# nv-tlabs/ChronoEdit

Measured on AMD Instinct MI355X. Metric: denoising-steps/sec, higher is better.
Workload: dtype bf16

## Files before the change

### chronoedit_amd/csrc/ce_attn.hip

```cpp
#include <cstdlib>

#include "ce_common.h"

namespace {

constexpr int HD = 128;
constexpr int QW = 32;
constexpr int KVB = 64;
constexpr int K_TILE_BYTES = KVB * HD * 2;
constexpr int VT_TILE_BYTES = HD * KVB * 2;
constexpr int BUF_BYTES = K_TILE_BYTES + VT_TILE_BYTES;
constexpr int OST_ROW = HD * 2 + 16;
constexpr int smem_bytes(int nwave, bool two_seg) {
  const int stage = nwave * QW * OST_ROW;
  return two_seg ? 2 * BUF_BYTES + stage : (stage > 2 * BUF_BYTES ? stage : 2 * BUF_BYTES);
}
constexpr float NEG_BIG = -1.0e30f;

__device__ __forceinline__ int vt_swz(int dv) {
  return ((((dv >> 2) & 7) << 1) | (((dv >> 1) ^ (dv >> 5)) & 1)) ^ (((dv >> 6) & 1) << 1);
}

struct KVSeg {
  const bf16* k;
// ... 220 lines not shown
          w1 = pack_bf16(bf16lo(pv[1]) + bf16lo(w1), bf16hi(pv[1]) + bf16hi(w1));
        }
        u32x2 val = {w0, w1};
        *slot = val;
      }
  }

  __syncthreads();
#pragma unroll
  for (int i = 0; i < 8; ++i) {
    const int c = lane + 64 * i;
    const int rl = c >> 4, cc = c & 15;
    const int q = q0 + rl;
    if (q < Nq) {
      const u32x4 v = *reinterpret_cast<const u32x4*>(smem + (TWO_SEG ? 2 * BUF_BYTES : 0) + (size_t)(wave * QW + rl) * OST_ROW + cc * 16);
      *reinterpret_cast<u32x4*>(O + (size_t)q * ldo + hoff + cc * 8) = v;
    }
  }
}


#define CE_EPOCH_BARRIER()                          \
  asm volatile("s_waitcnt lgkmcnt(0)" ::: "memory"); \
  __builtin_amdgcn_s_barrier()
constexpr int PK_ROW = HD * 2 + 16;
constexpr int PV_ROW = KVB * 2 + 16;
constexpr int PK_TILE = KVB * PK_ROW;
constexpr int PV_TILE = HD * PV_ROW;
typedef __attribute__((ext_vector_type(4))) unsigned pp_u4;
typedef __attribute__((ext_vector_type(2))) unsigned pp_u2;

constexpr int K_GRP = 1088;
typedef __attribute__((address_space(3))) void lds_void;
#ifdef CE_DIAGNOSTICS
__device__ unsigned long long g_sp_exact_hits = 0ull;
#endif
constexpr float SP_SPEC_THR = 1024.0f;
constexpr int SP_V0 = 2 * PK_TILE;
constexpr int SP_TILE_BYTES = 2 * PK_TILE + 3 * PV_TILE;
constexpr int sp_smem_bytes(bool two_seg) { return two_seg ? SP_TILE_BYTES + 8 * QW * OST_ROW : SP_TILE_BYTES; }

template <bool TWO_SEG, bool VT = false, bool QOUT = false, bool WGT = false>
__global__ __launch_bounds__(512, 2) void attn_fwd_sp_kernel(const bf16* __restrict__ Q_, bf16* __restrict__ O_, KVSeg seg0_,
                                                              KVSeg seg1_, int Nq, int H, int ldq, int ldo, int nqb,
                                                              float scale_log2e, int batch, BlkRows blk) {
  extern __shared__ __attribute__((aligned(16))) unsigned char smem[];
  constexpr int NWAVE = 8, QB = QW * NWAVE;
  const int tid = threadIdx.x, lane = tid & 63;
  const int wave = __builtin_amdgcn_readfirstlane(tid >> 6);
  const int l31 = lane & 31, hh = lane >> 5;
  for (int item = blockIdx.x; item < nqb * H * batch; item += gridDim.x) {
  const bf16* Q = Q_;
  bf16* O = O_;
  KVSeg seg0 = seg0_, seg1 = seg1_;

  int head, qb, bz;
  {
    const int nqb_full = Nq / QB;
    if ((H & 7) == 0) {
      const int xcd = item & 7, local = item >> 3, hx_n = H >> 3;
      const int full = batch * hx_n * nqb_full;
      if (local < full) {
        bz = local / (hx_n * nqb_full);
        const int r = local % (hx_n * nqb_full);
        head = xcd + 8 * (r / nqb_full);
        qb = r % nqb_full;
      } else {
        const int l2 = local - full;
        bz = l2 / hx_n;
        head = xcd + 8 * (l2 % hx_n);
        qb = nqb_full;
      }
    } else {
      bz = item / (nqb * H);
      const int r = item % (nqb * H);
      head = r / nqb;
      qb = r % nqb;
    }
  }
  {
    if (VT && blk.rows > 0) {
      Q += (size_t)bz * blk.rows * ldq;
      O += (size_t)bz * blk.rows * ldo;
      seg0.k += (size_t)bz * blk.rows * seg0.ldk;
      seg0.v += (size_t)bz * blk.vt_cols;
    } else if (TWO_SEG && VT) {
      Q += (size_t)bz * blk.q_rows * ldq;
      O += (size_t)bz * Nq * ldo;
      seg0.k += (size_t)bz * blk.k0_rows * seg0.ldk;
      seg0.v += (size_t)bz * blk.vt_cols;
    } else {
      Q += (size_t)bz * Nq * ldq;
      O += (size_t)bz * Nq * ldo;
      seg0.k += (size_t)bz * seg0.len * seg0.ldk;
      seg0.v += VT ? (size_t)bz * (TWO_SEG ? blk.vt_cols : seg0.len) : (size_t)bz * seg0.len * seg0.ldv;
    }
    if (TWO_SEG) {
      seg1.k += (size_t)bz * (VT ? blk.k1_rows : seg1.len) * seg1.ldk;
      seg1.v += VT ? (size_t)bz * blk.stride : (size_t)bz * seg1.len * seg1.ldv;
    }
  }
  const int q0 = qb * QB + wave * QW;
  const int hoff = head * HD;
  const bool active = q0 < Nq;
  const int q0row = (VT && blk.rows > 0) ? (q0 / blk.rows) * blk.stride + q0 % blk.rows : q0;

  bf16x8 qf[8];
  {
    const bf16* qrow = Q + (size_t)(q0 + l31 < Nq ? q0row + l31 : 0) * ldq + hoff + 8 * hh;
#pragma unroll
    for (int ks = 0; ks < 8; ++ks) qf[ks] = *reinterpret_cast<const bf16x8*>(qrow + 16 * ks);
  }
  auto scale_q = [&]() __attribute__((always_inline)) {
#pragma unroll
  for (int ks = 0; ks < 8; ++ks) {
    const u32x4 w = __builtin_bit_cast(u32x4, qf[ks]);
    u32x4 o;
#pragma unroll
    for (int i = 0; i < 4; ++i) o[i] = pack_bf16(bf16lo(w[i]) * scale_log2e, bf16hi(w[i]) * scale_log2e);
    qf[ks] = __builtin_bit_cast(bf16x8, o);
  }
#pragma unroll
  for (int ks = 0; ks < 8; ++ks) asm volatile("" : "+v"(qf[ks]));

  };
  const int v_dvq = (tid & 1) | (((tid >> 4) & 15) << 1), v_kvq = ((tid >> 1) & 7) | (((tid >> 8) & 1) << 3);
  const int v_chunk = (v_kvq & ~3) | ((v_kvq & 1) << 1) | ((v_kvq >> 1) & 1);
  unsigned char* ost = smem + (TWO_SEG ? SP_TILE_BYTES : 0) + (size_t)(wave * QW + l31) * OST_ROW;
  const int k_w = l31 & 3;
  const unsigned char* k_rd = smem + (l31 >> 2) * K_GRP + k_w * 256 + ((hh ^ (k_w & 1)) << 4);
  const int k_eo[2] = {(k_w >> 1) << 5, ((k_w >> 1) ^ 1) << 5};
  const unsigned char* v_rd = smem + SP_V0 + l31 * PV_ROW + hh * 16;
  int vt_off[4];
#pragma unroll
  for (int s4 = 0; s4 < 4; ++s4) {
    const int x = (l31 >> 1) & 7;
    vt_off[s4] = l31 * 128 + ((2 * (s4 ^ (x >> 1)) + (hh ^ (x & 1))) << 4);
  }
  unsigned char* v_wr = smem + SP_V0 + (4 * v_dvq) * PV_ROW + v_chunk * 8;

#pragma unroll
  for (int sidx = 0; sidx < (TWO_SEG ? 2 : 1); ++sidx) {
    KVSeg sg = sidx == 0 ? seg0 : seg1;
    float w_last = 0.f;
    if (WGT && sidx == 0) {
      sg.len = min(max(blk.valid0[bz], 1), sg.len);
      w_last = blk.w0[bz];
    }
    const int ntiles = (sg.len + KVB - 1) / KVB;
    const int k_rows_span = (VT && blk.rows > 0) ? ((sg.len - 1) / blk.rows) * blk.stride + blk.rows : sg.len;
    const auto k_rsrc = __builtin_amdgcn_make_buffer_rsrc((void*)(sg.k + hoff), 0, (k_rows_span - 1) * sg.ldk * 2 + HD * 2, 0x00020000);
    const auto v_rsrc = VT ? __builtin_amdgcn_make_buffer_rsrc((void*)(sg.v + (size_t)hoff * sg.ldv), 0, ((HD - 1) * sg.ldv + ntiles * KVB) * 2, 0x00020000)
                           : __builtin_amdgcn_make_buffer_rsrc((void*)(sg.v + hoff), 0, (sg.len - 1) * sg.ldv * 2 + HD * 2, 0x00020000);
    int v_voff[4];
#pragma unroll
    for (int i = 0; i < 4; ++i) v_voff[i] = (4 * v_kvq + i) * sg.ldv * 2 + v_dvq * 8;
    const int k_tile_bytes = KVB * sg.ldk * 2, v_tile_bytes = KVB * sg.ldv * 2;

    f32x16 oacc[4];
#pragma unroll
    for (int m = 0; m < 4; ++m)
#pragma unroll
      for (int r = 0; r < 16; ++r) oacc[m][r] = 0.f;
    float l_run = 0.f, alpha_prev = 1.0f, mc = 0.f;
    f32x16 cinit;
#pragma unroll
    for (int r = 0; r < 16; ++r) cinit[r] = 0.f;
    u32x4 ppk[4];
#pragma unroll
    for (int s4 = 0; s4 < 4; ++s4) ppk[s4] = u32x4{0u, 0u, 0u, 0u};

    pp_u2 vreg[4];
    const int kd_row = VT ? (lane >> 4) + 4 * ((wave >> 1) & 1) + 8 * (wave & 1) + 16 * (wave >> 2) : 4 * wave + (lane >> 4);
    const int kd_voff0 = kd_row * sg.ldk * 2 + (((lane & 15) ^ (lane >> 4)) << 4), kd_voff1 = kd_voff0 + 32 * sg.ldk * 2;
    const int vd_row = 8 * wave + (lane >> 3);
    const int vd_voff0 = vd_row * sg.ldv * 2 + (((lane & 7) ^ ((vd_row >> 1) & 7)) << 4), vd_voff1 = vd_voff0 + 64 * sg.ldv * 2;
    auto dma_v = [&](int t, int buf, int j) {
      __builtin_amdgcn_raw_ptr_buffer_load_lds(v_rsrc, (lds_void*)(smem + SP_V0 + buf * PV_TILE + (wave + 8 * j) * 1024), 16,
                                               j ? vd_voff1 : vd_voff0, t * (KVB * 2), 0, 0);
    };
    auto dma_k = [&](int t, int buf, int j) {
      int soff = t * k_tile_bytes;
      if (VT && blk.rows > 0) {
        const int b_ = blk.magic ? (int)__umulhi((uint32_t)t, blk.magic) : t;
        soff = (b_ * blk.stride + (t - b_ * (blk.rows >> 6)) * KVB) * sg.ldk * 2;
      }
      __builtin_amdgcn_raw_ptr_buffer_load_lds(k_rsrc, (lds_void*)(smem + buf * PK_TILE + (wave + 8 * j) * K_GRP), 16,
                                               j ? kd_voff1 : kd_voff0, soff, 0, 0);
    };
    auto load_v = [&](int t) {
      const int so = t * v_tile_bytes;
#pragma unroll
      for (int i = 0; i < 4; ++i) vreg[i] = __builtin_amdgcn_raw_buffer_load_b64(v_rsrc, v_voff[i], so, 0);
    };
    auto store_v_part = [&](int buf, int j) {
      const int w = j >> 1;
      uint32_t lo, hi;
      if ((j & 1) == 0) {
        lo = (vreg[0][w] & 0xffffu) | (vreg[1][w] << 16);
        hi = (vreg[2][w] & 0xffffu) | (vreg[3][w] << 16);
      } else {
        lo = (vreg[0][w] >> 16) | (vreg[1][w] & 0xffff0000u);
        hi = (vreg[2][w] >> 16) | (vreg[3][w] & 0xffff0000u);
      }
      pp_u2 val = {lo, hi};
      *reinterpret_cast<pp_u2*>(v_wr + buf * PV_TILE + j * PV_ROW) = val;
    };
    auto store_v = [&](int buf) {
#pragma unroll
      for (int j = 0; j < 4; ++j) {
        const int w = j >> 1;
        uint32_t lo, hi;
        if ((j & 1) == 0) {
          lo = (vreg[0][w] & 0xffffu) | (vreg[1][w] << 16);
          hi = (vreg[2][w] & 0xffffu) | (vreg[3][w] << 16);
        } else {
          lo = (vreg[0][w] >> 16) | (vreg[1][w] & 0xffff0000u);
          hi = (vreg[2][w] >> 16) | (vreg[3][w] & 0xffff0000u);
        }
        pp_u2 val = {lo, hi};
        *reinterpret_cast<pp_u2*>(v_wr + buf * PV_TILE + j * PV_ROW) = val;
      }
    };

    if (TWO_SEG && sidx == 1) { CE_EPOCH_BARRIER(); }
    dma_k(0, 0, 0);
    dma_k(0, 0, 1);
    __builtin_amdgcn_sched_barrier(0);
    if (VT) {
      dma_v(0, 0, 0);
      dma_v(0, 0, 1);
    } else {
      load_v(0);
    }
    {
      const pp_u4 z = {0u, 0u, 0u, 0u};
      for (int i = tid; i < PV_TILE / 16; i += NWAVE * 64) *reinterpret_cast<pp_u4*>(smem + SP_V0 + 2 * PV_TILE + i * 16) = z;
    }
    if (!VT) {
      store_v(0);
      asm volatile("s_waitcnt vmcnt(0)" ::: "memory");
      load_v(1);
    }
    if (sidx == 0) scale_q();

#define CE_SP_KWAIT()                                          \
  do {                                                         \
    if (VT) asm volatile("s_waitcnt vmcnt(2)" ::: "memory");   \
    else asm volatile("s_waitcnt vmcnt(4)" ::: "memory");      \
  } while (0)
    int vb_prev = 2, vb_cur = 0;

    for (int t = 0; !active && t < ntiles; ++t) {
      CE_SP_KWAIT();
      CE_EPOCH_BARRIER();
      const int vb_next = 3 - vb_prev - vb_cur;
      dma_k(t + 1, (t + 1) & 1, 0);
      dma_k(t + 1, (t + 1) & 1, 1);
      __builtin_amdgcn_sched_barrier(0);
      if (VT) {
        dma_v(t + 1, vb_next, 0);
        dma_v(t + 1, vb_next, 1);
      } else {
        store_v(vb_next);
        load_v(t + 2);
      }
      vb_prev = vb_cur;
      vb_cur = vb_next;
    }
    for (int t = 0; active && t < ntiles; ++t) {
      CE_SP_KWAIT();
      CE_EPOCH_BARRIER();
      const int vb_next = 3 - vb_prev - vb_cur;
      const unsigned char* kb = k_rd + (t & 1) * PK_TILE;
      const unsigned char* vb = v_rd + vb_prev * PV_TILE;
      const unsigned char* vtb = smem + SP_V0 + vb_prev * PV_TILE;

      const f32x16 zero16 = {0.f, 0.f, 0.f, 0.f, 0.f, 0.f, 0.f, 0.f, 0.f, 0.f, 0.f, 0.f, 0.f, 0.f, 0.f, 0.f};
      f32x16 st[2];
      {
        constexpr int RING = VT ? 4 : 6;
        bf16x8 kf[RING];
#define CE_LDK(i) (*reinterpret_cast<const bf16x8*>(kb + k_eo[((i) >> 1) & 1] + ((i) & 1) * 8 * K_GRP + ((i) >> 2) * 64))
#pragma unroll
        for (int i = 0; i < RING; ++i) kf[i] = CE_LDK(i);
#pragma unroll
        for (int i = 0; i < 16; ++i) {
          if (i < 2) {
            asm("v_mfma_f32_32x32x16_bf16 %0, %1, %2, %3" : "=&v"(st[i & 1]) : "v"(kf[i % RING]), "v"(qf[i >> 1]), "v"(cinit));
          } else {
            st[i & 1] = __builtin_amdgcn_mfma_f32_32x32x16_bf16(kf[i % RING], qf[i >> 1], st[i & 1], 0, 0, 0);
          }
          if (i + RING < 16) kf[i % RING] = CE_LDK(i + RING);
          if (i == 1) dma_k(t + 1, (t + 1) & 1, 0);
          if (i == 3) dma_k(t + 1, (t + 1) & 1, 1);
          if (VT) {
            if (i == 5) dma_v(t + 1, vb_next, 0);
            if (i == 7) dma_v(t + 1, vb_next, 1);
          } else {
            if (i == 12) load_v(t + 2);
            if (i >= 5 && i < 9) store_v_part(vb_next, i - 5);
          }
          __builtin_amdgcn_sched_barrier(0);
        }
#undef CE_LDK
      }
      float alpha = 1.0f;
      float psum = 0.f;
      auto mask_tail = [&]() {
        if ((t + 1) * KVB > sg.len) {
          int thr = sg.len - t * KVB - (VT ? 8 : 4) * hh;
          asm volatile("" : "+v"(thr));
#pragma unroll
          for (int f = 0; f < 2; ++f)
#pragma unroll
            for (int r = 0; r < 16; ++r) {
              const int c = VT ? 32 * f + 16 * (r >> 3) + 4 * ((r >> 2) & 1) + (r & 3)
                               : 32 * f + (r & 3) + 8 * (r >> 2);
              if (c >= thr) st[f][r] = NEG_BIG;
            }
        }
      };
      auto weigh_last = [&]() {
        if (WGT && sidx == 0 && t == ntiles - 1 && w_last != 0.f) {
          int pos = sg.len - 1 - t * KVB - 8 * hh;
          asm volatile("" : "+v"(pos));
#pragma unroll
          for (int f = 0; f < 2; ++f)
#pragma unroll
            for (int r = 0; r < 16; ++r) {
              const int c = 32 * f + 16 * (r >> 3) + 4 * ((r >> 2) & 1) + (r & 3);
// ... 62 lines not shown
          __builtin_amdgcn_sched_barrier(0);
        }
        psum += st[1][14];
        psum += st[1][15];
#pragma unroll
        for (int j = 12; j < 16; ++j) pack_pair(j);
#undef CE_LDV
      }
      if (__builtin_expect(t > 0 && __any(psum > SP_SPEC_THR), 0)) {
        CE_DIAG_COUNT_EXACT(g_sp_exact_hits);
#pragma unroll
        for (int i = 0; i < 16; ++i) {
          const bf16x8 kfr = *reinterpret_cast<const bf16x8*>(kb + k_eo[(i >> 1) & 1] + (i & 1) * 8 * K_GRP + (i >> 2) * 64);
          st[i & 1] = __builtin_amdgcn_mfma_f32_32x32x16_bf16(kfr, qf[i >> 1], i < 2 ? zero16 : st[i & 1], 0, 0, 0);
        }
#pragma unroll
        for (int f = 0; f < 2; ++f)
#pragma unroll
          for (int r = 0; r < 16; ++r) st[f][r] -= mc;
        mask_tail();
        weigh_last();
        rebase();
        psum = 0.f;
#pragma unroll
        for (int j = 0; j < 16; ++j) {
          st[j >> 3][(2 * j) & 15] = __builtin_amdgcn_exp2f(st[j >> 3][(2 * j) & 15]);
          st[j >> 3][(2 * j + 1) & 15] = __builtin_amdgcn_exp2f(st[j >> 3][(2 * j + 1) & 15]);
          psum += st[j >> 3][(2 * j) & 15] + st[j >> 3][(2 * j + 1) & 15];
          pack_pair(j);
        }
      }
      l_run = l_run * alpha + psum;
      alpha_prev = alpha;
      vb_prev = vb_cur;
      vb_cur = vb_next;
    }
    if (active && __any(alpha_prev != 1.0f)) {
#pragma unroll
      for (int m = 0; m < 4; ++m)
#pragma unroll
        for (int r = 0; r < 16; ++r) oacc[m][r] *= alpha_prev;
    }
    if (VT) {
      asm volatile("s_waitcnt vmcnt(0)" ::: "memory");
      __builtin_amdgcn_s_barrier();
    }
    if (active) {
      const unsigned char* vb = v_rd + vb_prev * PV_TILE;
      const unsigned char* vtb = smem + SP_V0 + vb_prev * PV_TILE;
#pragma unroll
      for (int u = 0; u < 16; ++u) {
        const bf16x8 vfd = VT ? *reinterpret_cast<const bf16x8*>(vtb + vt_off[u >> 2] + (u & 3) * 4096)
                              : *reinterpret_cast<const bf16x8*>(vb + (u & 3) * 32 * PV_ROW + (u >> 2) * 32);
        oacc[u & 3] = __builtin_amdgcn_mfma_f32_32x32x16_bf16(vfd, __builtin_bit_cast(bf16x8, ppk[u >> 2]), oacc[u & 3], 0, 0, 0);
      }
    }
    CE_EPOCH_BARRIER();

    const float l_tot = l_run + __shfl_xor(l_run, 32, 64);
    const float inv = 1.0f / l_tot;
#pragma unroll
    for (int m = 0; m < 4; ++m)
#pragma unroll
      for (int a = 0; a < 4; ++a) {
        uint32_t w0 = pack_bf16(oacc[m][4 * a + 0] * inv, oacc[m][4 * a + 1] * inv);
        uint32_t w1 = pack_bf16(oacc[m][4 * a + 2] * inv, oacc[m][4 * a + 3] * inv);
        u32x2* slot = reinterpret_cast<u32x2*>(ost + (32 * m + 8 * a + 4 * hh) * 2);
        if (TWO_SEG && sidx == 1) {
          const u32x2 pv = *slot;
          w0 = pack_bf16(bf16lo(pv[0]) + bf16lo(w0), bf16hi(pv[0]) + bf16hi(w0));
          w1 = pack_bf16(bf16lo(pv[1]) + bf16lo(w1), bf16hi(pv[1]) + bf16hi(w1));
        }
        u32x2 val = {w0, w1};
        *slot = val;
      }
  }

  if (TWO_SEG && VT && QOUT) {
    const int ktiles = (H * HD) >> 7;
    const int grow = bz * Nq + q0 + l31;
#pragma unroll
    for (int m = 0; m < 4; ++m) {
      uint32_t pk[8];
      float amax = 0.f;
#pragma unroll
      for (int a = 0; a < 4; ++a) {
        const u32x2 pv = *reinterpret_cast<const u32x2*>(ost + (32 * m + 8 * a + 4 * hh) * 2);
        pk[2 * a] = pv[0];
        pk[2 * a + 1] = pv[1];
        amax = fmaxf(amax, fmaxf(fmaxf(fabsf(bf16lo(pv[0])), fabsf(bf16hi(pv[0]))), fmaxf(fabsf(bf16lo(pv[1])), fabsf(bf16hi(pv[1])))));
      }
      amax = fmaxf(amax, __shfl_xor(amax, 32, 64));
      const int byte = mx_scale_byte_nosat(amax);
      const float is = mx_inv_scale(byte);
#pragma unroll
      for (int a = 0; a < 4; ++a) {
        int w = 0;
        w = __builtin_amdgcn_cvt_pk_fp8_f32(clamp448(bf16lo(pk[2 * a]) * is), clamp448(bf16hi(pk[2 * a]) * is), w, false);
        w = __builtin_amdgcn_cvt_pk_fp8_f32(clamp448(bf16lo(pk[2 * a + 1]) * is), clamp448(bf16hi(pk[2 * a + 1]) * is), w, true);
        *reinterpret_cast<uint32_t*>(ost + 32 * m + 8 * a + 4 * hh) = (uint32_t)w;
      }
      if (hh == 0 && q0 + l31 < Nq) blk.s8[mx_gemm_scale_offset(grow, head * 4 + m, ktiles)] = (unsigned char)byte;
    }
    __syncthreads();
    unsigned char* O8 = blk.q8 + (size_t)bz * Nq * blk.ld8;
#pragma unroll
    for (int i = 0; i < 4; ++i) {
      const int c = lane + 64 * i;
      const int rl = c >> 3, cc = c & 7;
      if (q0 + rl < Nq) {
        const u32x4 v = *reinterpret_cast<const u32x4*>(smem + SP_TILE_BYTES + (size_t)(wave * QW + rl) * OST_ROW + cc * 16);
        *reinterpret_cast<u32x4*>(O8 + (size_t)(q0 + rl) * blk.ld8 + hoff + cc * 16) = v;
      }
    }
  } else {
  __syncthreads();
#pragma unroll
  for (int i = 0; i < 8; ++i) {
    const int c = lane + 64 * i;
    const int rl = c >> 4, cc = c & 15;
    if (q0 + rl < Nq) {
      const u32x4 v = *reinterpret_cast<const u32x4*>(smem + (TWO_SEG ? SP_TILE_BYTES : 0) + (size_t)(wave * QW + rl) * OST_ROW + cc * 16);
      *reinterpret_cast<u32x4*>(O + (size_t)(q0row + rl) * ldo + hoff + cc * 8) = v;
    }
  }
  }
  __syncthreads();
  }
}


#define W4A_S_FIRST(ST, KF, QF, CI) asm volatile("v_mfma_f32_32x32x16_bf16 %0, %1, %2, %3" : "=&v"(ST) : "v"(KF), "a"(QF), "v"(CI))
#define W4A_S(ST, KF, QF) asm volatile("v_mfma_f32_32x32x16_bf16 %0, %1, %2, %0" : "+v"(ST) : "v"(KF), "a"(QF))
#define W4A_PV(OA, VF, PP) asm volatile("v_mfma_f32_32x32x16_bf16 %0, %1, %2, %0" : "+a"(OA) : "v"(VF), "v"(PP))
#define W4A_ADD(ACC, X) asm volatile("v_add_f32 %0, %0, %1" : "+v"(ACC) : "v"(X))
#define W4A_CVT(DST, A, B)                                                                  \
  do {                                                                                      \
    uint32_t w_;                                                                            \
    asm volatile("v_cvt_pk_bf16_f32 %0, %1, %2" : "=v"(w_) : "v"(A), "v"(B));               \
    (DST) = w_;                                                                             \
  } while (0)
#ifndef W4_KDMA_IN_PV
#define W4_KDMA_IN_PV 1
#endif
#ifndef W4_ABLATE
#define W4_ABLATE 0
#endif
#ifndef W4_EXP_ASM
#define W4_EXP_ASM 1
#endif
#if W4_EXP_ASM
#define W4A_EXP(X) asm volatile("v_exp_f32 %0, %0" : "+v"(X))
#else
#define W4A_EXP(X) (X) = __builtin_amdgcn_exp2f(X)
#endif
#define W4A_SETTLE_S(SB) asm volatile("s_nop 11" : "+v"(st[SB][0]), "+v"(st[SB][1]))
#define W4A_SETTLE_O(SB) asm volatile("s_nop 11" : "+a"(oacc[SB][0]), "+a"(oacc[SB][1]), "+a"(oacc[SB][2]), "+a"(oacc[SB][3]))
constexpr int W4_KB = 4;
constexpr int W4_V0 = W4_KB * PK_TILE;
constexpr int W4_SMEM = W4_V0 + 3 * PV_TILE;
template <int N>
struct w4_int {
// ... 459 lines not shown
#ifdef CE_DIAGNOSTICS
extern "C" int ce_diag_mx_exact_hits(unsigned long long* out, int reset);
CE_API int ce_diag_attention_exact_route_hits(unsigned long long* hits, int reset) {
  if (!hits) return CE_ERR_ARG;
  unsigned long long v = 0ull, z = 0ull;
  if (hipDeviceSynchronize() != hipSuccess) return CE_ERR_ARG;
  if (hipMemcpyFromSymbol(&v, HIP_SYMBOL(g_sp_exact_hits), sizeof(v)) != hipSuccess) return CE_ERR_ARG;
  if (reset && hipMemcpyToSymbol(HIP_SYMBOL(g_sp_exact_hits), &z, sizeof(z)) != hipSuccess) return CE_ERR_ARG;
  hits[0] = v;
  return ce_diag_mx_exact_hits(hits + 1, reset);
}
#endif
CE_KNOB g_attn_nwave = 0;
#ifdef CE_DIAGNOSTICS
CE_API int ce_set_attention_waves(int nwave) {
  const int old = g_attn_nwave;
  if (nwave == 0 || nwave == 4 || nwave == 8 || nwave == 16 || nwave == 64 || nwave == 128 || nwave == 129) g_attn_nwave = nwave;
  return old;
}
#endif

CE_API int ce_attention_batched_bf16(const void* Q, const void* K1, const void* V1, int len1, int ldk1, int ldv1,
                                         const void* K2, const void* V2, int len2, int ldk2, int ldv2, void* O, int Nq, int H,
                                         int head_dim, int ldq, int ldo, float softmax_scale, int batch, hipStream_t stream) {
  if (!Q || !K1 || !V1 || !O) return CE_ERR_ARG;
  if (head_dim != HD || Nq <= 0 || H <= 0 || len1 <= 0 || batch <= 0 || batch > 65535) return CE_ERR_SHAPE;
  if ((ldq & 7) || (ldo & 7) || (ldk1 & 7) || (ldv1 & 3)) return CE_ERR_ALIGN;
  const bool two = (K2 != nullptr && V2 != nullptr && len2 > 0);
  if (two && ((ldk2 & 7) || (ldv2 & 3))) return CE_ERR_ALIGN;
  KVSeg s0{(const bf16*)K1, (const bf16*)V1, len1, ldk1, ldv1};
  KVSeg s1{(const bf16*)K2, (const bf16*)V2, two ? len2 : 0, ldk2, ldv2};
  const float sl2 = softmax_scale * 1.4426950408889634f;
  const bool sp = g_attn_nwave == 64 || g_attn_nwave == 0 || g_attn_nwave >= 128;
  const int nwave = sp ? 8 : g_attn_nwave;
  const int nqb = (Nq + nwave * QW - 1) / (nwave * QW);
  dim3 grid(nqb * H, batch), block(nwave * 64);
  if (sp) {
#define CE_ATTN_SP(TWO)                                                                                              \
  do {                                                                                                               \
    static bool done_[CE_MAX_DEVICES] = {};                                                                          \
    bool& done = done_[ce_device_slot()];                                                                            \
    if (!done) {                                                                                                     \
      (void)hipFuncSetAttribute((const void*)attn_fwd_sp_kernel<TWO>, hipFuncAttributeMaxDynamicSharedMemorySize,    \
                                sp_smem_bytes(TWO));                                                                 \
      done = true;                                                                                                   \
    }                                                                                                                \
    hipLaunchKernelGGL((attn_fwd_sp_kernel<TWO>), dim3(nqb * H * batch), block, sp_smem_bytes(TWO), stream, (const bf16*)Q, \
                       (bf16*)O, s0, s1, Nq, H, ldq, ldo, nqb, sl2, batch, BlkRows{0, 0, 0u, 0});                    \
  } while (0)
    if (two) CE_ATTN_SP(true); else CE_ATTN_SP(false);
#undef CE_ATTN_SP
    return (int)hipGetLastError();
  }
#define CE_ATTN_LAUNCH(TWO, NW)                                                                                     \
  do {                                                                                                              \
    static bool done_[CE_MAX_DEVICES] = {};                                                                         \
    bool& done = done_[ce_device_slot()];                                                                           \
    if (!done) {                                                                                                    \
      (void)hipFuncSetAttribute((const void*)attn_fwd_kernel<TWO, NW>, hipFuncAttributeMaxDynamicSharedMemorySize,  \
                                smem_bytes(NW, TWO));                                                               \
      done = true;                                                                                                  \
    }                                                                                                               \
    hipLaunchKernelGGL((attn_fwd_kernel<TWO, NW>), grid, block, smem_bytes(NW, TWO), stream, (const bf16*)Q, (bf16*)O, \
                       s0, s1, Nq, H, ldq, ldo, nqb, sl2);                                                          \
  } while (0)
  if (two) {
// ... 22 lines not shown

CE_API int ce_v_transpose_blocked_bf16(const void* v, int ldv, void* vt, int ldvt, int n_keys, int H, int batch, int blk_rows, int blk_stride,
                                           int vt_sample_cols, hipStream_t stream) {
  if (!v || !vt) return CE_ERR_ARG;
  if (n_keys <= 0 || H <= 0 || batch <= 0 || blk_rows <= 0 || (blk_rows & 63) || blk_stride < batch * blk_rows || (vt_sample_cols & 63) ||
      vt_sample_cols < (n_keys + KVB - 1) / KVB * KVB || ldvt < batch * vt_sample_cols)
    return CE_ERR_SHAPE;
  if ((ldv & 3) || (ldvt & 7)) return CE_ERR_ALIGN;
  hipLaunchKernelGGL(v_transpose_kernel, dim3(vt_sample_cols / KVB, H, batch), dim3(256), 0, stream, (const bf16*)v, ldv, (bf16*)vt, ldvt, n_keys,
                     blk_rows, blk_stride, vt_sample_cols);
  return (int)hipGetLastError();
}

#ifdef CE_DIAGNOSTICS
extern "C" int ce_attn16_launch(const void* Q, const void* K, const void* Vt, int len, int ldk, int ldvt, void* O, int Nq, int H, int ldq, int ldo,
                                float sl2, int batch, int cus, hipStream_t stream);
#endif

static int attention_vt_launch(const void* Q, const void* K, const void* Vt, int len, int ldk, int ldvt, void* O, int Nq, int H, int head_dim,
                               int ldq, int ldo, float softmax_scale, int batch, int blk_rows, int blk_stride, int vt_sample_cols,
                               hipStream_t stream) {
  if (!Q || !K || !Vt || !O) return CE_ERR_ARG;
  if (head_dim != HD || Nq <= 0 || H <= 0 || len <= 0 || batch <= 0 || batch > 65535) return CE_ERR_SHAPE;
  const int ntiles_cols = (len + KVB - 1) / KVB * KVB;
  if (blk_rows == 0) {
    vt_sample_cols = len;
    if (ldvt < (batch - 1) * len + ntiles_cols) return CE_ERR_SHAPE;
  } else {
    if ((blk_rows & 63) || blk_stride < batch * blk_rows || (Nq % blk_rows) || vt_sample_cols < ntiles_cols ||
        ldvt < (batch - 1) * vt_sample_cols + ntiles_cols)
      return CE_ERR_SHAPE;
  }
  if ((ldq & 7) || (ldo & 7) || (ldk & 7) || (ldvt & 7) || (batch > 1 && (vt_sample_cols & 1))) return CE_ERR_ALIGN;
  KVSeg s0{(const bf16*)K, (const bf16*)Vt, len, ldk, ldvt};
  KVSeg s1{nullptr, nullptr, 0, 0, 0};
  BlkRows blk{blk_rows, blk_stride, 0u, vt_sample_cols};
  if (blk_rows > 0) {
    const uint32_t tps = (uint32_t)(blk_rows >> 6);
    blk.magic = tps == 1 ? 0u : (uint32_t)(((1ull << 32) + tps - 1) / tps);
  }
  const float sl2 = softmax_scale * 1.4426950408889634f;
  const int nqb = (Nq + 8 * QW - 1) / (8 * QW);
  static bool done_[CE_MAX_DEVICES] = {};
  bool& done = done_[ce_device_slot()];
  if (!done) {
    (void)hipFuncSetAttribute((const void*)attn_fwd_sp_kernel<false, true>, hipFuncAttributeMaxDynamicSharedMemorySize, sp_smem_bytes(false));
    done = true;
  }
  const int cus = ce_device_cus();
  const int items = nqb * H * batch;
#ifdef CE_DIAGNOSTICS
  if (g_attn_nwave == 16 && blk_rows == 0) {
    const int rc = ce_attn16_launch(Q, K, Vt, len, ldk, ldvt, O, Nq, H, ldq, ldo, sl2, batch, cus, stream);
    if (rc != CE_ERR_ALIGN) return rc;
  }
#endif
  if (g_attn_nwave == 128 || g_attn_nwave == 129) {
    static bool done4_[CE_MAX_DEVICES] = {};
    bool& done4 = done4_[ce_device_slot()];
    if (!done4) {
      (void)hipFuncSetAttribute((const void*)attn_fwd_w4_kernel, hipFuncAttributeMaxDynamicSharedMemorySize, W4_SMEM);
      done4 = true;
    }
    const int grid4 = (g_attn_nwave == 129 && items > cus) ? (cus & ~7) : items;
    hipLaunchKernelGGL(attn_fwd_w4_kernel, dim3(grid4), dim3(256), W4_SMEM, stream, (const bf16*)Q, (bf16*)O, s0, Nq, H, ldq, ldo, nqb,
                       sl2, batch, blk);
// ... 4 lines not shown
                     s0, s1, Nq, H, ldq, ldo, nqb, sl2, batch, blk);
  return (int)hipGetLastError();
}

CE_API int ce_attention_vt_bf16(const void* Q, const void* K, const void* Vt, int len, int ldk, int ldvt, void* O, int Nq, int H,
                                    int head_dim, int ldq, int ldo, float softmax_scale, int batch, hipStream_t stream) {
  return attention_vt_launch(Q, K, Vt, len, ldk, ldvt, O, Nq, H, head_dim, ldq, ldo, softmax_scale, batch, 0, 0, 0, stream);
}

CE_API int ce_attention_vt_blocked_bf16(const void* Q, const void* K, const void* Vt, int len, int ldk, int ldvt, void* O, int Nq, int H,
                                            int head_dim, int ldq, int ldo, float softmax_scale, int batch, int blk_rows, int blk_stride,
                                            int vt_sample_cols, hipStream_t stream) {
  if (blk_rows <= 0) return CE_ERR_SHAPE;
  return attention_vt_launch(Q, K, Vt, len, ldk, ldvt, O, Nq, H, head_dim, ldq, ldo, softmax_scale, batch, blk_rows, blk_stride, vt_sample_cols,
                             stream);
}


static int attention_2seg_vt_launch(const void* Q, const void* K1, const void* V1t, int len1, int ldk1, int ldv1t, int vt_cols1,
                                    const void* K2, const void* V2t, int len2, int ldk2, int ldv2t, int vt_cols2, void* O, int Nq,
                                    int H, int head_dim, int ldq, int ldo, float softmax_scale, int batch, void* O8, void* S8, int ldo8,
                                    int q_rows, int k1_rows, int k2_rows, hipStream_t stream, const void* valid1 = nullptr,
                                    const void* w1 = nullptr) {
  if (!Q || !K1 || !V1t || !K2 || !V2t || (!O && !O8)) return CE_ERR_ARG;
  if ((valid1 != nullptr) != (w1 != nullptr) || (valid1 && O8)) return CE_ERR_ARG;
  if ((q_rows != 0 && q_rows < Nq) || (k1_rows != 0 && k1_rows < len1) || (k2_rows != 0 && k2_rows < len2)) return CE_ERR_SHAPE;
  if (k1_rows == 0) vt_cols1 = 0;
  if (k2_rows == 0) vt_cols2 = 0;
  if (head_dim != HD || Nq <= 0 || H <= 0 || len1 <= 0 || len2 <= 0 || batch <= 0 || batch > 65535) return CE_ERR_SHAPE;
  const int c1 = (len1 + KVB - 1) / KVB * KVB, c2 = (len2 + KVB - 1) / KVB * KVB;
  if ((k1_rows != 0 && vt_cols1 < len1) || (k2_rows != 0 && vt_cols2 < len2) || ldv1t < (batch - 1) * vt_cols1 + c1 || ldv2t < (batch - 1) * vt_cols2 + c2)
    return CE_ERR_SHAPE;
  if ((ldq & 7) || (ldo & 7) || (ldk1 & 7) || (ldk2 & 7) || (ldv1t & 7) || (ldv2t & 7) || (vt_cols1 & 1) || (vt_cols2 & 1)) return CE_ERR_ALIGN;
  KVSeg s0{(const bf16*)K1, (const bf16*)V1t, len1, ldk1, ldv1t};
  KVSeg s1{(const bf16*)K2, (const bf16*)V2t, len2, ldk2, ldv2t};
  const float sl2 = softmax_scale * 1.4426950408889634f;
  const int nqb = (Nq + 8 * QW - 1) / (8 * QW);
  static bool done_[CE_MAX_DEVICES] = {};
  bool& done = done_[ce_device_slot()];
  if (!done) {
    (void)hipFuncSetAttribute((const void*)attn_fwd_sp_kernel<true, true>, hipFuncAttributeMaxDynamicSharedMemorySize, sp_smem_bytes(true));
    (void)hipFuncSetAttribute((const void*)attn_fwd_sp_kernel<true, true, true>, hipFuncAttributeMaxDynamicSharedMemorySize, sp_smem_bytes(true));
    (void)hipFuncSetAttribute((const void*)attn_fwd_sp_kernel<true, true, false, true>, hipFuncAttributeMaxDynamicSharedMemorySize, sp_smem_bytes(true));
    done = true;
  }
  const BlkRows blk{0, vt_cols2, 0u, vt_cols1, (unsigned char*)O8, (unsigned char*)S8, ldo8, q_rows, k1_rows, k2_rows,
                    (const int*)valid1, (const float*)w1};
  const int cus = ce_device_cus();
  const int items = nqb * H * batch;
  const int grid = items <= 2 * cus ? items : ((2 * cus) & ~7);
  if (valid1)
    hipLaunchKernelGGL((attn_fwd_sp_kernel<true, true, false, true>), dim3(grid), dim3(512), sp_smem_bytes(true), stream, (const bf16*)Q,
                       (bf16*)O, s0, s1, Nq, H, ldq, ldo, nqb, sl2, batch, blk);
  else if (O8)
    hipLaunchKernelGGL((attn_fwd_sp_kernel<true, true, true>), dim3(grid), dim3(512), sp_smem_bytes(true), stream, (const bf16*)Q,
                       (bf16*)O, s0, s1, Nq, H, ldq, ldo, nqb, sl2, batch, blk);
  else
    hipLaunchKernelGGL((attn_fwd_sp_kernel<true, true>), dim3(grid), dim3(512), sp_smem_bytes(true), stream, (const bf16*)Q, (bf16*)O,
                       s0, s1, Nq, H, ldq, ldo, nqb, sl2, batch, blk);
  return (int)hipGetLastError();
}

CE_API int ce_attention_2seg_vt_bf16(const void* Q, const void* K1, const void* V1t, int len1, int ldk1, int ldv1t, int vt_cols1,
                                         const void* K2, const void* V2t, int len2, int ldk2, int ldv2t, int vt_cols2, void* O, int Nq,
                                         int H, int head_dim, int ldq, int ldo, float softmax_scale, int batch, hipStream_t stream) {
  if (!O) return CE_ERR_ARG;
// ... 31 lines not shown
```

Measured before the change: 3.109.

## Prefetch next segment/item K/V tiles and Q across persistent attention loop

In the persistent VT attention kernel, the first K/V tiles of the next segment or next work item are now DMA'd into LDS during the last tile of the current one. The next item's Q rows are loaded early, before the output epilogue. Both changes remove the pipeline drain and refill bubble at segment and item boundaries, and some barriers are dropped. In exchange the kernel always reserves the output staging LDS, carries buffer-index state across iterations, and adds a leading-dimension limit check because offsets are now computed with 24-bit multiplies.

```diff
diff --git a/chronoedit_amd/csrc/ce_attn.hip b/chronoedit_amd/csrc/ce_attn.hip
--- a/chronoedit_amd/csrc/ce_attn.hip
+++ b/chronoedit_amd/csrc/ce_attn.hip
@@ -276,13 +276,22 @@
 
 constexpr int K_GRP = 1088;
 typedef __attribute__((address_space(3))) void lds_void;
+typedef const __attribute__((address_space(4))) int* const_int_p;
+typedef const __attribute__((address_space(4))) float* const_float_p;
 #ifdef CE_DIAGNOSTICS
 __device__ unsigned long long g_sp_exact_hits = 0ull;
 #endif
 constexpr float SP_SPEC_THR = 1024.0f;
 constexpr int SP_V0 = 2 * PK_TILE;
 constexpr int SP_TILE_BYTES = 2 * PK_TILE + 3 * PV_TILE;
-constexpr int sp_smem_bytes(bool two_seg) { return two_seg ? SP_TILE_BYTES + 8 * QW * OST_ROW : SP_TILE_BYTES; }
+constexpr int sp_smem_bytes(bool) { return SP_TILE_BYTES + 8 * QW * OST_ROW; }
+constexpr int SP_MAX_LD = 1 << 23;
+
+#if defined(__HIP_DEVICE_COMPILE__)
+#define CE_LDS_DMA16(RSRC, LDS, VOFF, SOFF) __builtin_amdgcn_raw_ptr_buffer_load_lds(RSRC, LDS, 16, VOFF, SOFF, 0, 0)
+#else
+#define CE_LDS_DMA16(RSRC, LDS, VOFF, SOFF) ((void)0)
+#endif
 
 template <bool TWO_SEG, bool VT = false, bool QOUT = false, bool WGT = false>
 __global__ __launch_bounds__(512, 2) void attn_fwd_sp_kernel(const bf16* __restrict__ Q_, bf16* __restrict__ O_, KVSeg seg0_,
@@ -293,65 +302,116 @@
   const int tid = threadIdx.x, lane = tid & 63;
   const int wave = __builtin_amdgcn_readfirstlane(tid >> 6);
   const int l31 = lane & 31, hh = lane >> 5;
-  for (int item = blockIdx.x; item < nqb * H * batch; item += gridDim.x) {
-  const bf16* Q = Q_;
-  bf16* O = O_;
-  KVSeg seg0 = seg0_, seg1 = seg1_;
-
-  int head, qb, bz;
-  {
+  const int n_items = nqb * H * batch;
+  int kcur = 0;
+  int vb_prev = 2, vb_cur = 0;
+  bf16x8 qf[8];
+  if (VT) {
+    const pp_u4 z = {0u, 0u, 0u, 0u};
+    for (int i = tid; i < PV_TILE / 16; i += NWAVE * 64) *reinterpret_cast<pp_u4*>(smem + SP_V0 + 2 * PV_TILE + i * 16) = z;
+  }
+  auto locate = [&](int it, int& head_, int& qb_, int& bz_) __attribute__((always_inline)) {
     const int nqb_full = Nq / QB;
     if ((H & 7) == 0) {
-      const int xcd = item & 7, local = item >> 3, hx_n = H >> 3;
+      const int xcd = it & 7, local = it >> 3, hx_n = H >> 3;
       const int full = batch * hx_n * nqb_full;
       if (local < full) {
-        bz = local / (hx_n * nqb_full);
+        bz_ = local / (hx_n * nqb_full);
         const int r = local % (hx_n * nqb_full);
-        head = xcd + 8 * (r / nqb_full);
-        qb = r % nqb_full;
+        head_ = xcd + 8 * (r / nqb_full);
+        qb_ = r % nqb_full;
       } else {
         const int l2 = local - full;
-        bz = l2 / hx_n;
-        head = xcd + 8 * (l2 % hx_n);
-        qb = nqb_full;
+        bz_ = l2 / hx_n;
+        head_ = xcd + 8 * (l2 % hx_n);
+        qb_ = nqb_full;
       }
     } else {
-      bz = item / (nqb * H);
-      const int r = item % (nqb * H);
-      head = r / nqb;
-      qb = r % nqb;
-    }
-  }
-  {
-    if (VT && blk.rows > 0) {
-      Q += (size_t)bz * blk.rows * ldq;
-      O += (size_t)bz * blk.rows * ldo;
-      seg0.k += (size_t)bz * blk.rows * seg0.ldk;
-      seg0.v += (size_t)bz * blk.vt_cols;
-    } else if (TWO_SEG && VT) {
-      Q += (size_t)bz * blk.q_rows * ldq;
-      O += (size_t)bz * Nq * ldo;
-      seg0.k += (size_t)bz * blk.k0_rows * seg0.ldk;
-      seg0.v += (size_t)bz * blk.vt_cols;
+      bz_ = it / (nqb * H);
+      const int r = it % (nqb * H);
+      head_ = r / nqb;
+      qb_ = r % nqb;
+    }
+  };
+  auto seg_of = [&](int sidx_, int bz_) __attribute__((always_inline)) {
+    KVSeg s = sidx_ == 0 ? seg0_ : seg1_;
+    if (sidx_ == 0) {
+      if (VT && blk.rows > 0) {
+        s.k += (size_t)bz_ * blk.rows * s.ldk;
+        s.v += (size_t)bz_ * blk.vt_cols;
+      } else if (TWO_SEG && VT) {
+        s.k += (size_t)bz_ * blk.k0_rows * s.ldk;
+        s.v += (size_t)bz_ * blk.vt_cols;
+      } else {
+        s.k += (size_t)bz_ * s.len * s.ldk;
+        s.v += VT ? (size_t)bz_ * (TWO_SEG ? blk.vt_cols : s.len) : (size_t)bz_ * s.len * s.ldv;
+      }
+      if (WGT) s.len = min(max(((const_int_p)blk.valid0)[bz_], 1), s.len);
     } else {
-      Q += (size_t)bz * Nq * ldq;
-      O += (size_t)bz * Nq * ldo;
-      seg0.k += (size_t)bz * seg0.len * seg0.ldk;
-      seg0.v += VT ? (size_t)bz * (TWO_SEG ? blk.vt_cols : seg0.len) : (size_t)bz * seg0.len * seg0.ldv;
-    }
-    if (TWO_SEG) {
-      seg1.k += (size_t)bz * (VT ? blk.k1_rows : seg1.len) * seg1.ldk;
-      seg1.v += VT ? (size_t)bz * blk.stride : (size_t)bz * seg1.len * seg1.ldv;
-    }
-  }
+      s.k += (size_t)bz_ * (VT ? blk.k1_rows : s.len) * s.ldk;
+      s.v += VT ? (size_t)bz_ * blk.stride : (size_t)bz_ * s.len * s.ldv;
+    }
+    return s;
+  };
+  auto k_rows_span = [&](const KVSeg& s) __attribute__((always_inline)) {
+    return (VT && blk.rows > 0) ? ((s.len - 1) / blk.rows) * blk.stride + blk.rows : s.len;
+  };
+#define CE_K_DESC(S, HOFF) __builtin_amdgcn_make_buffer_rsrc((void*)((S).k + (HOFF)), 0, (k_rows_span(S) - 1) * (S).ldk * 2 + HD * 2, 0x00020000)
+#define CE_V_DESC(S, HOFF)                                                                                                                 \
+  (VT ? __builtin_amdgcn_make_buffer_rsrc((void*)((S).v + (size_t)(HOFF) * (S).ldv), 0, ((HD - 1) * (S).ldv + ((S).len + KVB - 1) / KVB * KVB) * 2, \
+                                          0x00020000)                                                                                      \
+      : __builtin_amdgcn_make_buffer_rsrc((void*)((S).v + (HOFF)), 0, ((S).len - 1) * (S).ldv * 2 + HD * 2, 0x00020000))
+  auto q_rows = [&](int bz_, int qb_, int head_) __attribute__((always_inline)) {
+    const int srows = (VT && blk.rows > 0) ? blk.rows : (TWO_SEG && VT) ? blk.q_rows : Nq;
+    const int q0_ = qb_ * QB + wave * QW;
+    const int q0row_ = (VT && blk.rows > 0) ? (q0_ / blk.rows) * blk.stride + q0_ % blk.rows : q0_;
+    return Q_ + (size_t)bz_ * srows * ldq + (size_t)(q0_ + l31 < Nq ? q0row_ + l31 : 0) * ldq + head_ * HD + 8 * hh;
+  };
+
+  const int kd_row = VT ? (lane >> 4) + 4 * ((wave >> 1) & 1) + 8 * (wave & 1) + 16 * (wave >> 2) : 4 * wave + (lane >> 4);
+  const int vd_row = 8 * wave + (lane >> 3);
+  const int kd_chunk = ((lane & 15) ^ (lane >> 4)) << 4, vd_chunk = ((lane & 7) ^ ((vd_row >> 1) & 7)) << 4;
+#define CE_FETCH_K0(RSRC, LDK, BUF, J)                                                       \
+  CE_LDS_DMA16(RSRC, (lds_void*)(smem + (BUF) * PK_TILE + (wave + 8 * (J)) * K_GRP),         \
+               kd_row * (LDK) * 2 + kd_chunk + (J) * 32 * (LDK) * 2, 0)
+#define CE_FETCH_V0(RSRC, LDV, BUF, J)                                                       \
+  CE_LDS_DMA16(RSRC, (lds_void*)(smem + SP_V0 + (BUF) * PV_TILE + (wave + 8 * (J)) * 1024),  \
+               vd_row * (LDV) * 2 + vd_chunk + (J) * 64 * (LDV) * 2, 0)
+  if (VT && (int)blockIdx.x < n_items) {
+    int head_, qb_, bz_;
+    locate(blockIdx.x, head_, qb_, bz_);
+    const bf16* qrow = q_rows(bz_, qb_, head_);
+#pragma unroll
+    for (int ks = 0; ks < 8; ++ks) qf[ks] = *reinterpret_cast<const bf16x8*>(qrow + 16 * ks);
+    const KVSeg s0 = seg_of(0, bz_);
+    {
+      const auto k0_rsrc = CE_K_DESC(s0, head_ * HD);
+      const auto v0_rsrc = CE_V_DESC(s0, head_ * HD);
+      CE_FETCH_K0(k0_rsrc, s0.ldk, 0, 0);
+      CE_FETCH_K0(k0_rsrc, s0.ldk, 0, 1);
+      __builtin_amdgcn_sched_barrier(0);
+      CE_FETCH_V0(v0_rsrc, s0.ldv, 0, 0);
+      CE_FETCH_V0(v0_rsrc, s0.ldv, 0, 1);
+      __builtin_amdgcn_sched_barrier(0);
+    }
+#pragma unroll
+    for (int ks = 0; ks < 8; ++ks) asm volatile("" : "+v"(qf[ks]));
+    asm volatile("s_waitcnt vmcnt(2)" ::: "memory");
+  }
+  for (int item = blockIdx.x; item < n_items; item += gridDim.x) {
+  int head, qb, bz;
+  locate(item, head, qb, bz);
+  const bool more = VT && item + (int)gridDim.x < n_items;
+  int head_n = head, qb_n = qb, bz_n = bz;
+  if (more) locate(item + (int)gridDim.x, head_n, qb_n, bz_n);
+  bf16* O = O_ + (size_t)bz * ((VT && blk.rows > 0) ? blk.rows : Nq) * ldo;
   const int q0 = qb * QB + wave * QW;
   const int hoff = head * HD;
   const bool active = q0 < Nq;
   const int q0row = (VT && blk.rows > 0) ? (q0 / blk.rows) * blk.stride + q0 % blk.rows : q0;
 
-  bf16x8 qf[8];
-  {
-    const bf16* qrow = Q + (size_t)(q0 + l31 < Nq ? q0row + l31 : 0) * ldq + hoff + 8 * hh;
+  if (!VT) {
+    const bf16* qrow = q_rows(bz, qb, head);
 #pragma unroll
     for (int ks = 0; ks < 8; ++ks) qf[ks] = *reinterpret_cast<const bf16x8*>(qrow + 16 * ks);
   }
@@ -370,7 +430,7 @@
   };
   const int v_dvq = (tid & 1) | (((tid >> 4) & 15) << 1), v_kvq = ((tid >> 1) & 7) | (((tid >> 8) & 1) << 3);
   const int v_chunk = (v_kvq & ~3) | ((v_kvq & 1) << 1) | ((v_kvq >> 1) & 1);
-  unsigned char* ost = smem + (TWO_SEG ? SP_TILE_BYTES : 0) + (size_t)(wave * QW + l31) * OST_ROW;
+  unsigned char* ost = smem + SP_TILE_BYTES + (size_t)(wave * QW + l31) * OST_ROW;
   const int k_w = l31 & 3;
   const unsigned char* k_rd = smem + (l31 >> 2) * K_GRP + k_w * 256 + ((hh ^ (k_w & 1)) << 4);
   const int k_eo[2] = {(k_w >> 1) << 5, ((k_w >> 1) ^ 1) << 5};
@@ -385,17 +445,18 @@
 
 #pragma unroll
   for (int sidx = 0; sidx < (TWO_SEG ? 2 : 1); ++sidx) {
-    KVSeg sg = sidx == 0 ? seg0 : seg1;
-    float w_last = 0.f;
-    if (WGT && sidx == 0) {
-      sg.len = min(max(blk.valid0[bz], 1), sg.len);
-      w_last = blk.w0[bz];
-    }
+    constexpr int NSEG = TWO_SEG ? 2 : 1;
+    const bool last_seg = sidx == NSEG - 1;
+    const KVSeg sg = seg_of(sidx, bz);
+    const float w_last = (WGT && sidx == 0) ? ((const_float_p)blk.w0)[bz] : 0.f;
     const int ntiles = (sg.len + KVB - 1) / KVB;
-    const int k_rows_span = (VT && blk.rows > 0) ? ((sg.len - 1) / blk.rows) * blk.stride + blk.rows : sg.len;
-    const auto k_rsrc = __builtin_amdgcn_make_buffer_rsrc((void*)(sg.k + hoff), 0, (k_rows_span - 1) * sg.ldk * 2 + HD * 2, 0x00020000);
-    const auto v_rsrc = VT ? __builtin_amdgcn_make_buffer_rsrc((void*)(sg.v + (size_t)hoff * sg.ldv), 0, ((HD - 1) * sg.ldv + ntiles * KVB) * 2, 0x00020000)
-                           : __builtin_amdgcn_make_buffer_rsrc((void*)(sg.v + hoff), 0, (sg.len - 1) * sg.ldv * 2 + HD * 2, 0x00020000);
+    const auto k_rsrc = CE_K_DESC(sg, hoff);
+    const auto v_rsrc = CE_V_DESC(sg, hoff);
+    const bool hand = VT && (!last_seg || more);
+    const KVSeg ng = !VT ? sg : !last_seg ? seg_of(sidx + 1, bz) : more ? seg_of(0, bz_n) : sg;
+    const int hoff_x = (VT && last_seg && more) ? head_n * HD : hoff;
+    const auto nk_rsrc = CE_K_DESC(ng, hoff_x);
+    const auto nv_rsrc = CE_V_DESC(ng, hoff_x);
     int v_voff[4];
 #pragma unroll
     for (int i = 0; i < 4; ++i) v_voff[i] = (4 * v_kvq + i) * sg.ldv * 2 + v_dvq * 8;
@@ -415,23 +476,24 @@
     for (int s4 = 0; s4 < 4; ++s4) ppk[s4] = u32x4{0u, 0u, 0u, 0u};
 
     pp_u2 vreg[4];
-    const int kd_row = VT ? (lane >> 4) + 4 * ((wave >> 1) & 1) + 8 * (wave & 1) + 16 * (wave >> 2) : 4 * wave + (lane >> 4);
-    const int kd_voff0 = kd_row * sg.ldk * 2 + (((lane & 15) ^ (lane >> 4)) << 4), kd_voff1 = kd_voff0 + 32 * sg.ldk * 2;
-    const int vd_row = 8 * wave + (lane >> 3);
-    const int vd_voff0 = vd_row * sg.ldv * 2 + (((lane & 7) ^ ((vd_row >> 1) & 7)) << 4), vd_voff1 = vd_voff0 + 64 * sg.ldv * 2;
-    auto dma_v = [&](int t, int buf, int j) {
-      __builtin_amdgcn_raw_ptr_buffer_load_lds(v_rsrc, (lds_void*)(smem + SP_V0 + buf * PV_TILE + (wave + 8 * j) * 1024), 16,
-                                               j ? vd_voff1 : vd_voff0, t * (KVB * 2), 0, 0);
-    };
-    auto dma_k = [&](int t, int buf, int j) {
+    auto fetch_k = [&](bool nx, int t, int buf, int j) {
       int soff = t * k_tile_bytes;
       if (VT && blk.rows > 0) {
         const int b_ = blk.magic ? (int)__umulhi((uint32_t)t, blk.magic) : t;
         soff = (b_ * blk.stride + (t - b_ * (blk.rows >> 6)) * KVB) * sg.ldk * 2;
       }
-      __builtin_amdgcn_raw_ptr_buffer_load_lds(k_rsrc, (lds_void*)(smem + buf * PK_TILE + (wave + 8 * j) * K_GRP), 16,
-                                               j ? kd_voff1 : kd_voff0, soff, 0, 0);
+      const int pitch = (nx ? ng.ldk : sg.ldk) * 2;
+      CE_LDS_DMA16(nx ? nk_rsrc : k_rsrc, (lds_void*)(smem + buf * PK_TILE + (wave + 8 * j) * K_GRP),
+                   (int)__umul24(kd_row, pitch) + kd_chunk + j * 32 * pitch, nx ? 0 : soff);
     };
+    auto fetch_v = [&](bool nx, int t, int buf, int j) {
+      const int pitch = (nx ? ng.ldv : sg.ldv) * 2;
+      CE_LDS_DMA16(nx ? nv_rsrc : v_rsrc, (lds_void*)(smem + SP_V0 + buf * PV_TILE + (wave + 8 * j) * 1024),
+                   (int)__umul24(vd_row, pitch) + vd_chunk + j * 64 * pitch, nx ? 0 : t * (KVB * 2));
+    };
+    auto dma_k = [&](int t, int buf, int j) { fetch_k(false, t, buf, j); };
+    auto next_k = [&](bool pf, int t, int buf, int j) { fetch_k(pf, t + 1, buf, j); };
+    auto next_v = [&](bool pf, int t, int buf, int j) { fetch_v(pf, t + 1, buf, j); };
     auto load_v = [&](int t) {
       const int so = t * v_tile_bytes;
 #pragma unroll
@@ -467,56 +529,55 @@
       }
     };
 
-    if (TWO_SEG && sidx == 1) { CE_EPOCH_BARRIER(); }
-    dma_k(0, 0, 0);
-    dma_k(0, 0, 1);
-    __builtin_amdgcn_sched_barrier(0);
-    if (VT) {
-      dma_v(0, 0, 0);
-      dma_v(0, 0, 1);
-    } else {
+    const bool from_item = VT && sidx == 0;
+    if (!VT) {
+      if (TWO_SEG && sidx == 1) { CE_EPOCH_BARRIER(); }
+      kcur = 0, vb_prev = 2, vb_cur = 0;
+      dma_k(0, 0, 0);
+      dma_k(0, 0, 1);
+      __builtin_amdgcn_sched_barrier(0);
       load_v(0);
-    }
-    {
-      const pp_u4 z = {0u, 0u, 0u, 0u};
-      for (int i = tid; i < PV_TILE / 16; i += NWAVE * 64) *reinterpret_cast<pp_u4*>(smem + SP_V0 + 2 * PV_TILE + i * 16) = z;
-    }
-    if (!VT) {
+      {
+        const pp_u4 z = {0u, 0u, 0u, 0u};
+        for (int i = tid; i < PV_TILE / 16; i += NWAVE * 64) *reinterpret_cast<pp_u4*>(smem + SP_V0 + 2 * PV_TILE + i * 16) = z;
+      }
       store_v(0);
       asm volatile("s_waitcnt vmcnt(0)" ::: "memory");
       load_v(1);
     }
     if (sidx == 0) scale_q();
 
-#define CE_SP_KWAIT()                                          \
-  do {                                                         \
-    if (VT) asm volatile("s_waitcnt vmcnt(2)" ::: "memory");   \
-    else asm volatile("s_waitcnt vmcnt(4)" ::: "memory");      \
+#define CE_SP_KWAIT(T)                                                  \
+  do {                                                                  \
+    if (!VT) asm volatile("s_waitcnt vmcnt(4)" ::: "memory");           \
+    else if (!(from_item && (T) == 0)) asm volatile("s_waitcnt vmcnt(2)" ::: "memory"); \
   } while (0)
-    int vb_prev = 2, vb_cur = 0;
 
     for (int t = 0; !active && t < ntiles; ++t) {
-      CE_SP_KWAIT();
+      CE_SP_KWAIT(t);
       CE_EPOCH_BARRIER();
       const int vb_next = 3 - vb_prev - vb_cur;
-      dma_k(t + 1, (t + 1) & 1, 0);
-      dma_k(t + 1, (t + 1) & 1, 1);
+      const bool pf = hand && t == ntiles - 1;
+      next_k(pf, t, kcur ^ 1, 0);
+      next_k(pf, t, kcur ^ 1, 1);
       __builtin_amdgcn_sched_barrier(0);
       if (VT) {
-        dma_v(t + 1, vb_next, 0);
-        dma_v(t + 1, vb_next, 1);
+        next_v(pf, t, vb_next, 0);
+        next_v(pf, t, vb_next, 1);
       } else {
         store_v(vb_next);
         load_v(t + 2);
       }
+      kcur ^= 1;
       vb_prev = vb_cur;
       vb_cur = vb_next;
     }
     for (int t = 0; active && t < ntiles; ++t) {
-      CE_SP_KWAIT();
+      CE_SP_KWAIT(t);
       CE_EPOCH_BARRIER();
       const int vb_next = 3 - vb_prev - vb_cur;
-      const unsigned char* kb = k_rd + (t & 1) * PK_TILE;
+      const bool pf = hand && t == ntiles - 1;
+      const unsigned char* kb = k_rd + kcur * PK_TILE;
       const unsigned char* vb = v_rd + vb_prev * PV_TILE;
       const unsigned char* vtb = smem + SP_V0 + vb_prev * PV_TILE;
 
@@ -536,11 +597,11 @@
             st[i & 1] = __builtin_amdgcn_mfma_f32_32x32x16_bf16(kf[i % RING], qf[i >> 1], st[i & 1], 0, 0, 0);
           }
           if (i + RING < 16) kf[i % RING] = CE_LDK(i + RING);
-          if (i == 1) dma_k(t + 1, (t + 1) & 1, 0);
-          if (i == 3) dma_k(t + 1, (t + 1) & 1, 1);
+          if (i == 1) next_k(pf, t, kcur ^ 1, 0);
+          if (i == 3) next_k(pf, t, kcur ^ 1, 1);
           if (VT) {
-            if (i == 5) dma_v(t + 1, vb_next, 0);
-            if (i == 7) dma_v(t + 1, vb_next, 1);
+            if (i == 5) next_v(pf, t, vb_next, 0);
+            if (i == 7) next_v(pf, t, vb_next, 1);
           } else {
             if (i == 12) load_v(t + 2);
             if (i >= 5 && i < 9) store_v_part(vb_next, i - 5);
@@ -669,9 +730,17 @@
       }
       l_run = l_run * alpha + psum;
       alpha_prev = alpha;
+      kcur ^= 1;
       vb_prev = vb_cur;
       vb_cur = vb_next;
     }
+    const bool q_ahead = VT && last_seg && more;
+    if (q_ahead) {
+      const bf16* qrow = q_rows(bz_n, qb_n, head_n);
+#pragma unroll
+      for (int ks = 0; ks < 8; ++ks) qf[ks] = *reinterpret_cast<const bf16x8*>(qrow + 16 * ks);
+      __builtin_amdgcn_sched_barrier(0);
+    }
     if (active && __any(alpha_prev != 1.0f)) {
 #pragma unroll
       for (int m = 0; m < 4; ++m)
@@ -679,7 +748,8 @@
         for (int r = 0; r < 16; ++r) oacc[m][r] *= alpha_prev;
     }
     if (VT) {
-      asm volatile("s_waitcnt vmcnt(0)" ::: "memory");
+      if (q_ahead) asm volatile("s_waitcnt vmcnt(12)" ::: "memory");
+      else asm volatile("s_waitcnt vmcnt(4)" ::: "memory");
       __builtin_amdgcn_s_barrier();
     }
     if (active) {
@@ -692,7 +762,7 @@
         oacc[u & 3] = __builtin_amdgcn_mfma_f32_32x32x16_bf16(vfd, __builtin_bit_cast(bf16x8, ppk[u >> 2]), oacc[u & 3], 0, 0, 0);
       }
     }
-    CE_EPOCH_BARRIER();
+    if (!VT) { CE_EPOCH_BARRIER(); }
 
     const float l_tot = l_run + __shfl_xor(l_run, 32, 64);
     const float inv = 1.0f / l_tot;
@@ -713,6 +783,15 @@
       }
   }
 
+  auto store_gate = [&]() __attribute__((always_inline)) {
+    if (VT) {
+      CE_EPOCH_BARRIER();
+#pragma unroll
+      for (int ks = 0; ks < 8; ++ks) asm volatile("" : "+v"(qf[ks]));
+    } else {
+      __syncthreads();
+    }
+  };
   if (TWO_SEG && VT && QOUT) {
     const int ktiles = (H * HD) >> 7;
     const int grow = bz * Nq + q0 + l31;
@@ -739,7 +818,7 @@
       }
       if (hh == 0 && q0 + l31 < Nq) blk.s8[mx_gemm_scale_offset(grow, head * 4 + m, ktiles)] = (unsigned char)byte;
     }
-    __syncthreads();
+    store_gate();
     unsigned char* O8 = blk.q8 + (size_t)bz * Nq * blk.ld8;
 #pragma unroll
     for (int i = 0; i < 4; ++i) {
@@ -751,20 +830,24 @@
       }
     }
   } else {
-  __syncthreads();
+  store_gate();
 #pragma unroll
   for (int i = 0; i < 8; ++i) {
     const int c = lane + 64 * i;
     const int rl = c >> 4, cc = c & 15;
     if (q0 + rl < Nq) {
-      const u32x4 v = *reinterpret_cast<const u32x4*>(smem + (TWO_SEG ? SP_TILE_BYTES : 0) + (size_t)(wave * QW + rl) * OST_ROW + cc * 16);
+      const u32x4 v = *reinterpret_cast<const u32x4*>(smem + SP_TILE_BYTES + (size_t)(wave * QW + rl) * OST_ROW + cc * 16);
       *reinterpret_cast<u32x4*>(O + (size_t)(q0row + rl) * ldo + hoff + cc * 8) = v;
     }
   }
   }
-  __syncthreads();
-  }
-}
+  if (!VT) __syncthreads();
+  }
+}
+#undef CE_FETCH_K0
+#undef CE_FETCH_V0
+#undef CE_K_DESC
+#undef CE_V_DESC
 
 
 #define W4A_S_FIRST(ST, KF, QF, CI) asm volatile("v_mfma_f32_32x32x16_bf16 %0, %1, %2, %3" : "=&v"(ST) : "v"(KF), "a"(QF), "v"(CI))
@@ -1290,6 +1373,7 @@
   KVSeg s1{(const bf16*)K2, (const bf16*)V2, two ? len2 : 0, ldk2, ldv2};
   const float sl2 = softmax_scale * 1.4426950408889634f;
   const bool sp = g_attn_nwave == 64 || g_attn_nwave == 0 || g_attn_nwave >= 128;
+  if (sp && (ldk1 >= SP_MAX_LD || (two && ldk2 >= SP_MAX_LD))) return CE_ERR_SHAPE;
   const int nwave = sp ? 8 : g_attn_nwave;
   const int nqb = (Nq + nwave * QW - 1) / (nwave * QW);
   dim3 grid(nqb * H, batch), block(nwave * 64);
@@ -1378,6 +1462,7 @@
       return CE_ERR_SHAPE;
   }
   if ((ldq & 7) || (ldo & 7) || (ldk & 7) || (ldvt & 7) || (batch > 1 && (vt_sample_cols & 1))) return CE_ERR_ALIGN;
+  if (ldk >= SP_MAX_LD || ldvt >= SP_MAX_LD) return CE_ERR_SHAPE;
   KVSeg s0{(const bf16*)K, (const bf16*)Vt, len, ldk, ldvt};
   KVSeg s1{nullptr, nullptr, 0, 0, 0};
   BlkRows blk{blk_rows, blk_stride, 0u, vt_sample_cols};
@@ -1448,6 +1533,7 @@
   if ((k1_rows != 0 && vt_cols1 < len1) || (k2_rows != 0 && vt_cols2 < len2) || ldv1t < (batch - 1) * vt_cols1 + c1 || ldv2t < (batch - 1) * vt_cols2 + c2)
     return CE_ERR_SHAPE;
   if ((ldq & 7) || (ldo & 7) || (ldk1 & 7) || (ldk2 & 7) || (ldv1t & 7) || (ldv2t & 7) || (vt_cols1 & 1) || (vt_cols2 & 1)) return CE_ERR_ALIGN;
+  if (ldk1 >= SP_MAX_LD || ldk2 >= SP_MAX_LD || ldv1t >= SP_MAX_LD || ldv2t >= SP_MAX_LD) return CE_ERR_SHAPE;
   KVSeg s0{(const bf16*)K1, (const bf16*)V1t, len1, ldk1, ldv1t};
   KVSeg s1{(const bf16*)K2, (const bf16*)V2t, len2, ldk2, ldv2t};
   const float sl2 = softmax_scale * 1.4426950408889634f;
```

New measurement: 3.108. No clear change (-0.0%).
